# Saguaro-Biosciences/image-processing-suite

Hardware: AMD Instinct MI355X
Metric: fields-of-view/sec, 2080x2080x5ch illum+seg+feat pipe (higher is better)
Workload: dtype fp32 planes / fp64 QC+features / fp32 CPnet (split-fp16 MFMA, f16x3); 1 GPU; configs[1]: 384-well plate, 1 FOV/well, 2080x2080x5ch, illum->seg->feat; batch_per_gpu=48, H=2080, W=2080, C=5, cellpose_model=nuclei, cpnet_weights=cpnet_nuclei_synth.pt, tiles_per_fov=9, parallelism=fov-sharded x1, scheduler=static per-rank steps, steps_this_rank=30, batches_in_flight_per_gpu=2

## Files before the change

image-processing-suite_amd/cpx/_lib.py:

```python
from __future__ import annotations

import ctypes as ct
import os
import threading

_HERE = os.path.dirname(os.path.abspath(__file__))
LIB_PATH = os.environ.get("CPX_LIB", os.path.join(_HERE, "libcpx.so"))

CPX_OK = 0
CPX_DTYPE_NONE, CPX_DTYPE_F32, CPX_DTYPE_F64, CPX_DTYPE_IMAGE_F64 = 0, 1, 2, 3
CPX_QC_OK, CPX_QC_FLAT, CPX_QC_NAN = 0, 1, 2

N_SHAPE = 15
N_INT = 5
N_TEX_PROPS = 6
N_ANGLES = 4
N_TEX = N_TEX_PROPS * N_ANGLES
FEATURES_PER_CHANNEL = N_INT + N_TEX
TEX_DISTANCE = 3


class CpxError(RuntimeError):
    """A libcpx entry point returned a non-zero status."""

# ... 84 lines not shown
    "cpx_seg_average": (_I, [_P, _P, _I, _I, _I, _P, _P, _P]),
    "cpx_embed_preprocess": (_I, [_P, _P, _P, _I, _I, _I, ct.c_float, ct.c_float, _P]),
    "cpx_effnet_stem": (_I, [_P, _P, _I, _I, _I, _P, _P, _P, _P]),
    "cpx_effnet_conv": (_I, [_P, _P, _I, _I, _I, _I, _I, _I, _I, _P, _P, _P, _I, _P, _P, _P]),
    "cpx_effnet_dw": (_I, [_P, _P, _I, _I, _I, _I, _I, _P, _P, _P, _P, _P]),
    "cpx_effnet_dw_blocks": (_I, [_I, _I, _I]),
    "cpx_effnet_se": (_I, [_P, _P, _I, _I, _I, _I, _I, _P, _P, _P, _P, _P]),
    "cpx_effnet_pool": (_I, [_P, _P, _I, _I, _I, _P]),
    "cpx_seg_masks": (_I, [_P, _P, _I, _P, _I, _I, _I, ct.c_double, _I, _I, _I, _P, _P]),
    "cpx_cpnet_epilogue": (_I, [_P, _P, _P, _P, _I, _P, _P, _P, _I, _I, _I, _I, _I, _P, _P, _I]),
    "cpx_cpnet_pool": (_I, [_P, _P, _P, _P, _I, _I, _I, _I, _I, _P, _P]),
    "cpx_cpnet_conv_cfg": (_I, [_I, _I, _P, _P]),
    "cpx_set_illum": (_I, [_P, _I, _P, _I, _I, _I]),
    "cpx_fov_submit": (_I, [_P, ct.c_int64, _P, _I, _I, _I, _I]),
    "cpx_fov_qc": (_I, [_P, _P, _P, _P]),
    "cpx_fov_planes": (_I, [_P, _P, _P]),
    "cpx_fov_read_plane": (_I, [_P, _I, _P]),
    "cpx_fov_segment_post": (_I, [_P, _P, _I, _P, _P, _I, ct.c_double, _I, _I, _I, _P, _P]),
    "cpx_fov_object_table": (_I, [_P, _P, _I, _I, _P, _P]),
    "cpx_fov_features": (_I, [_P, _P, _I, _P, _P]),
    "cpx_fov_wait": (_I, [_P]),
    "cpx_cpnet_conv3x3": (_I, [_P, _P, _I, _I, _I, _I, _I, _P, _P, _P, _I, _P, _P, _P, _I, _P, _P, _I]),
    "cpx_cpnet_conv3x3_head": (_I, [_P, _P, _I, _I, _I, _I, _I, _P, _P, _P, _I, _P, _P, _P, _I, _P,
                                    _P, _P, _I, _P]),
    "cpx_cpnet_stem": (_I, [_P, _P, _I, _I, _I, _P, _P, _P, _P, _P, _P, _P, _P, _P]),
    "cpx_cpnet_x3_cfg": (_I, [_I, _I, _I, _I, _P]),
    "cpx_cpnet_x3_conv": (_I, [_P, _I, _I, _P, _I, _I, _I, _I, _I, _I, _P, _P, _P, _I, _P, _I, _P, _P, _I,
                               _P, _P, _I, _P, _P, _I, _P, _P]),
    "cpx_cpnet_x3_conv_proj": (_I, [_P, _I, _P, _I, _I, _I, _I, _I, _P, _P, _I, _P, _P, _P, _I, _P, _P, _I,
                                    _P, _P, _I, _P]),
    "cpx_cpnet_x3_conv_pool": (_I, [_P, _I, _P, _I, _I, _I, _I, _I, _P, _P, _P, _P, _P, _P, _P, _P, _P]),
    "cpx_cpnet_x3_mask_overflow": (_I, [_P, _P, _I, _I, _I, _I, _P]),
    "cpx_cpnet_x3_stem": (_I, [_P, _P, _I, _I, _I, _P, _P, _P, _P, _P, _P, _P, _P, _P, _P]),
    "cpx_cpnet_x3_pool": (_I, [_P, _P, _P, _P, _I, _I, _I, _I, _I, _P, _P, _P]),
    "cpx_cpnet_x3_style": (_I, [_P, _P, _I, _I, _I, _I, _P, _P, _I, _P]),
}

_lib = None
_lock = threading.Lock()


def load(path: str | None = None):
    global _lib
    with _lock:
        if _lib is not None:
            return _lib
        p = path or LIB_PATH
        try:
            import torch
        except ImportError:
            pass
        if not os.path.exists(p):
            raise CpxNativeMissing(
                f"libcpx.so not found at {p}; build it with `python -c 'import __graft_entry__ as g; g.build()'`")
        try:
            lib = ct.CDLL(p)
        except OSError as e:
            raise CpxNativeMissing(f"failed to load {p}: {e}") from e
        for name, (res, args) in SIGNATURES.items():
            fn = getattr(lib, name)
            fn.restype = res
            fn.argtypes = args
        _lib = lib
        return lib


# ... 9 lines not shown
```

image-processing-suite_amd/cpx/cpnet_x3.py:

```python
from __future__ import annotations

import ctypes as ct

import numpy as np
import torch

from ._lib import check
from .cpnet import CPnet

X3_VARIANT = 0
X3_ZVARIANT = 3
X3_POOL_FUSE = True
X3_FOLD = True


def split_f16(w: np.ndarray):
    w = np.asarray(w, np.float32)
    if not np.all(np.abs(w) < 65504.0):
        raise ValueError("weights outside the fp16 range cannot be split")
    hi = w.astype(np.float16)
    lo = ((w - hi.astype(np.float32)) * np.float32(2048.0)).astype(np.float16)
    return hi, lo


def join_f16(hi: np.ndarray, lo: np.ndarray) -> np.ndarray:
    return (hi.astype(np.float32) + lo.astype(np.float32) * np.float32(1.0 / 2048.0)).astype(np.float32)


def pack_conv(w: np.ndarray, bm: int) -> np.ndarray:
    cout, cin, ks, _ = w.shape
    hi, lo = split_f16(w)
    parts = []
    for a in (hi, lo):
        t = a.reshape(cout // bm, bm, cin // 16, 16, ks, ks).transpose(0, 2, 4, 5, 1, 3)
        parts.append(t)
    return np.ascontiguousarray(np.stack(parts, axis=-2))


def to_split(x: np.ndarray) -> np.ndarray:
    hi, lo = split_f16(x)
    s = x.shape[:-1] + (x.shape[-1] // 16, 16)
    return np.ascontiguousarray(np.stack([hi.reshape(s), lo.reshape(s)], axis=-2))


def from_split(t: np.ndarray) -> np.ndarray:
    if t.dtype != np.float16:
# ... 143 lines not shown

    def _conv_pool(self, x, pk, cout, bias, res, bn):
        N, H, W, cin = x.shape
        yo = self._empty(N, H, W, cout)
        xo = self._empty(N, H // 2, W // 2, cout)
        zo = self._empty(N, H // 2, W // 2, cout)
        check(self.lib.cpx_cpnet_x3_conv_pool(
            self.dev.h, self.variant, _p(x), N, H, W, cin, cout, _p(pk), _p(bias), _p(res), _p(yo), _p(xo), _p(zo),
            _p(bn[0]), _p(bn[1]), self._ovf_p(N)), "cpx_cpnet_x3_conv_pool")
        return yo, xo, zo

    def _proj(self, x, blk):
        return self._conv(x, blk["wp"], blk["cout"], None, ks=1, relu=False, y=True, z=False)[0]

    def _pool(self, x, bn):
        N, H, W, C = x.shape
        xo = self._empty(N, H // 2, W // 2, C)
        zo = self._empty(N, H // 2, W // 2, C)
        scale, shift = bn
        check(self.lib.cpx_cpnet_x3_pool(self.dev.h, _p(x), _p(scale), _p(shift), 1, N, H // 2, W // 2, C,
                                         _p(xo), _p(zo), self._ovf_p(N)), "cpx_cpnet_x3_pool")
        return xo, zo

    def _stem(self, x, d):
        N, H, W, _ = x.shape
        p = self._empty(N, H, W, 32)
        z = self._empty(N, H, W, 32)
        (s0, h0), (s1, h1) = d["bn"][0], d["bn"][1]
        check(self.lib.cpx_cpnet_x3_stem(self.dev.h, _p(x), N, H, W, _p(s0), _p(h0), _p(d["stem_w"]),
                                         _p(d["b"][0]), _p(s1), _p(h1), _p(d["stem_wp"]), _p(p), _p(z),
                                         self._ovf_p(N)), "cpx_cpnet_x3_stem")
        return p, z

    def _style(self, x):
        N, H, W, C = x.shape
        S = torch.empty((N, self.J), dtype=torch.float32, device=self.td)
        check(self.lib.cpx_cpnet_x3_style(self.dev.h, _p(x), N, H, W, C, _p(self.lin_w), _p(self.lin_b),
                                          self.J, _p(S)), "cpx_cpnet_x3_style")
        return S

    @torch.no_grad()
    def __call__(self, x):
        self.dev._bind_stream()
        assert x.dtype == torch.float32 and x.is_contiguous() and x.shape[-1] == 2
        if self.ovf.numel() != x.shape[0]:
            self.ovf = torch.zeros(x.shape[0], dtype=torch.int32, device=self.td)
        self.ovf.zero_()
        xd = []
        zu = None
        nd = len(self.down)
        pooled = None
        for n, d in enumerate(self.down):
            if n == 0:
                p, z = self._stem(x, d)
                x1, z = self._conv(z, d["pk"][1], d["cout"], d["b1p"], res=p, bn=d["bn"][2], y=True)
            else:
                xin, z0 = pooled if pooled is not None else self._pool(xd[-1], d["bn"][0])
                _, z = self._conv(z0, d["pk"][0], d["cout"], d["b"][0], bn=d["bn"][1])
                if d["wpf"] is not None:
                    x1, z = self._conv_proj(z, d["pk"][1], d["cout"], d["b1p"], xin, d["wpf"], bn=d["bn"][2])
                else:
                    p = self._proj(xin, d)
                    x1, z = self._conv(z, d["pk"][1], d["cout"], d["b1p"], res=p, bn=d["bn"][2], y=True)
            _, z = self._conv(z, d["pk"][2], d["cout"], d["b"][2], bn=d["bn"][3])
            if n < nd - 1 and X3_POOL_FUSE:
                xo, xin_n, z0_n = self._conv_pool(z, d["pk"][3], d["cout"], d["b"][3], x1, self.down[n + 1]["bn"][0])
                pooled = (xin_n, z0_n)
            elif n < nd - 1:
                xo, _ = self._conv(z, d["pk"][3], d["cout"], d["b"][3], res=x1, y=True, z=False)
            else:
                xo, zu = self._conv(z, d["pk"][3], d["cout"], d["b"][3], res=x1, bn=self.up[-1]["bn"][0], y=True)
            xd.append(xo)
        S = self._style(xd[-1])
        J = self.J
        x_small, z0 = xd[-1], zu
        for n in range(len(self.up) - 1, -1, -1):
            u = self.up[n]
            so = self.style_off[n]
            sty = [(ct.c_void_p(S.data_ptr() + 4 * o), J) for o in so]
            p = None if u["wpf"] is not None else self._proj(x_small, u)
            _, z = self._conv(z0, u["pk"][0], u["cout"], u["b"][0], res=xd[n], style=sty[0], bn=u["bn"][1],
                              in_up=(n < len(self.up) - 1))
            if p is None:
                x1, z = self._conv_proj(z, u["pk"][1], u["cout"], u["b1p"], x_small, u["wpf"], style=sty[1],
                                        bn=u["bn"][2])
            else:
# ... 13 lines not shown
```

image-processing-suite_amd/csrc/k_conv_x3.hip:

```cpp
#include "cpx_internal.h"
#include <type_traits>
#include <stdlib.h>

namespace {

typedef _Float16 f16x8 __attribute__((ext_vector_type(8)));
typedef _Float16 f16x4 __attribute__((ext_vector_type(4)));
typedef float f32x16 __attribute__((ext_vector_type(16)));

constexpr float kLoScale = 2048.0f;
constexpr float kLoInv = 1.0f / 2048.0f;

typedef __attribute__((address_space(3))) void lds_void_t;
typedef __attribute__((address_space(1))) void glb_void_t;

__device__ uint4 g_x3_zero16 = {0u, 0u, 0u, 0u};

__device__ __forceinline__ int swz4(int row) { return (row >> 2) & 3; }

template <int Q>
__device__ __forceinline__ int swzq(int row) {
  if constexpr (Q >= 16) return row & 15;
  else if constexpr (Q == 8) return (row >> 1) & 7;
  else if constexpr (Q == 4) return (row >> 2) & 3;
// ... 2 lines not shown

__device__ __forceinline__ void split4(float a, float b, float c, float d, uint2& hi, uint2& lo, bool& bad) {
  const float v[4] = {a, b, c, d};
  f16x4 h, l;
#pragma unroll
  for (int k = 0; k < 4; ++k) {
    bad |= !(fabsf(v[k]) < 65504.0f);
    const float vc = fminf(fmaxf(v[k], -65504.0f), 65504.0f);
    const _Float16 t = (_Float16)vc;
    h[k] = t;
    l[k] = (_Float16)((vc - (float)t) * kLoScale);
  }
  hi = __builtin_bit_cast(uint2, h);
  lo = __builtin_bit_cast(uint2, l);
}

__device__ __forceinline__ void join4(const uint2& hi, const uint2& lo, float* out) {
  const f16x4 h = __builtin_bit_cast(f16x4, hi), l = __builtin_bit_cast(f16x4, lo);
#pragma unroll
  for (int k = 0; k < 4; ++k) out[k] = (float)h[k] + (float)l[k] * kLoInv;
}

__device__ __forceinline__ void join8(const uint4& hi, const uint4& lo, float* out) {
  join4(make_uint2(hi.x, hi.y), make_uint2(lo.x, lo.y), out);
  join4(make_uint2(hi.z, hi.w), make_uint2(lo.z, lo.w), out + 4);
}

__device__ __forceinline__ void split8(const float* v, uint4& hi, uint4& lo, bool& bad) {
  uint2 h0, l0, h1, l1;
  split4(v[0], v[1], v[2], v[3], h0, l0, bad);
  split4(v[4], v[5], v[6], v[7], h1, l1, bad);
  hi = make_uint4(h0.x, h0.y, h1.x, h1.y);
  lo = make_uint4(l0.x, l0.y, l1.x, l1.y);
}


struct X3Epi {
  const float* bias;
  const uint4* res;
  const float* style;
  const float* scale;
  const float* shift;
  uint4* y;
  uint4* z;
  int res_up, relu, z_up, style_stride;
  const float* head_w;
  const float* head_b;
  float* head;
  int n_head;
  int* ovf;
  int in_up;
  const uint4* in2;
  const uint4* wpk2;
  uint4* pool_x;
  uint4* pool_z;
  const float* pool_scale;
  const float* pool_shift;
};

template <int COUT, int BM, int TY, int TX, int WM, int WN>
__device__ __forceinline__ void x3_epilogue(f32x16 (&acc0)[WM][WN], const X3Epi& ep, uint4* smem, int n,
                                            int nb, int ty0, int tx0, int H, int W, int mw, int pg, int nsub,
                                            int tid = -1, uint4* res_lds = nullptr) {
  if (tid < 0) tid = threadIdx.x;
  uint4* const ybuf = smem;
  uint4* const zbuf = (res_lds && ep.y) ? res_lds : smem;
  constexpr int NT = 512;
  constexpr int P = TY * TX;
  constexpr int QB = BM / 4;
  constexpr int QC = COUT / 4;
  constexpr int OUT_R = (P * QB + NT - 1) / NT;
  const int lane = threadIdx.x & 63;
  const int h = lane >> 5, l32 = lane & 31;
  bool bad = false;
  auto gpix = [&](int px) -> long long {
    const int gy = ty0 + px / TX, gx = tx0 + px % TX;
    if (px >= P || gy >= H || gx >= W) return -1;
    return ((long long)n * H + gy) * W + gx;
  };
  auto slice = [&](int m) { return mw * WM + m; };
  auto piece = [&](const uint4* buf, int px, int m, int g, int lo) -> uint2* {
    const int q = (slice(m) * 2 + (g >> 1)) * 4 + 2 * lo + (g & 1);
    return reinterpret_cast<uint2*>(const_cast<uint4*>(buf) + px * QB + (q ^ swzq<QB>(px))) + h;
  };
  auto chan = [&](int m, int g) { return nb * BM + slice(m) * 32 + 8 * g + 4 * h; };
  if (ep.bias) {
#pragma unroll
    for (int m = 0; m < WM; ++m)
#pragma unroll
      for (int g = 0; g < 4; ++g) {
        const float4 bv = *reinterpret_cast<const float4*>(ep.bias + chan(m, g));
#pragma unroll
        for (int j = 0; j < WN; ++j) {
          acc0[m][j][4 * g + 0] += bv.x;
          acc0[m][j][4 * g + 1] += bv.y;
          acc0[m][j][4 * g + 2] += bv.z;
          acc0[m][j][4 * g + 3] += bv.w;
        }
      }
  }
  if (ep.res) {
    const uint4* rbuf = res_lds ? res_lds : smem;
    if (!res_lds) {
#pragma unroll
      for (int r = 0; r < OUT_R; ++r) {
        const int i = tid + r * NT;
        if (i < P * QB) {
          const int px = i / QB, k = i - px * QB;
          const int gy = ty0 + px / TX, gx = tx0 + px % TX;
          uint4 v = {0u, 0u, 0u, 0u};
          if (gy < H && gx < W) {
            const long long rp = ep.res_up ? ((long long)n * (H >> 1) + (gy >> 1)) * (W >> 1) + (gx >> 1)
                                           : ((long long)n * H + gy) * W + gx;
            v = ep.res[rp * QC + nb * QB + k];
          }
          smem[px * QB + (k ^ swzq<QB>(px))] = v;
        }
      }
      __syncthreads();
    }
#pragma unroll
    for (int j = 0; j < WN; ++j) {
      const int px = min((pg * WN + j) * 32 + l32, P - 1);
#pragma unroll
      for (int m = 0; m < WM; ++m)
#pragma unroll
        for (int g = 0; g < 4; ++g) {
          float rv[4];
          join4(*piece(rbuf, px, m, g, 0), *piece(rbuf, px, m, g, 1), rv);
#pragma unroll
          for (int k = 0; k < 4; ++k) acc0[m][j][4 * g + k] += rv[k];
        }
    }
    if (!res_lds) __syncthreads();
  }
  auto stage = [&](uint4* buf) {
// ... 433 lines not shown
#pragma unroll
              for (int m = 0; m < WM; ++m) {
                acc0[m][j] = __builtin_amdgcn_mfma_f32_32x32x16_f16(ah[m], bh, acc0[m][j], 0, 0, 0);
                acc1[m][j] = __builtin_amdgcn_mfma_f32_32x32x16_f16(ah[m], bl, acc1[m][j], 0, 0, 0);
                acc1[m][j] = __builtin_amdgcn_mfma_f32_32x32x16_f16(al[m], bh, acc1[m][j], 0, 0, 0);
              }
            }
          }
        }
      });
    }
    if (NBUF == 1) {
      __syncthreads();
      if (ch + 1 < NCHT) issue(ch + 1, 0);
    }
    asm volatile("s_waitcnt vmcnt(0)" ::: "memory");
    __syncthreads();
  }

#pragma unroll
  for (int m = 0; m < WM; ++m)
#pragma unroll
    for (int j = 0; j < WN; ++j)
#pragma unroll
      for (int r = 0; r < 16; ++r) acc0[m][j][r] += acc1[m][j][r] * kLoInv;

  if constexpr (kResPre)
    x3_epilogue<COUT, BM, TY, TX, WM, WN>(acc0, ep, bufO, n, nb, ty0, tx0, H, W, mw, pg, nsub, -1,
                                          ep.res ? bufR : nullptr);
  else
    x3_epilogue<COUT, BM, TY, TX, WM, WN>(acc0, ep, smem, n, nb, ty0, tx0, H, W, mw, pg, nsub);
}

template <int kP32Touch>
__global__ __launch_bounds__(512) __attribute__((amdgpu_waves_per_eu(4)))
void k_conv_x3_p32(const uint4* __restrict__ in, const uint4* __restrict__ wpk, X3Epi ep, int N, int H,
                   int W, int tiles_x, int tiles_y) {
  constexpr int NWV = 8, BM = 32, T = 9, TY = 8, TX = 32, HX = TX + 2, NPIX = (TY + 2) * HX;
  constexpr int NCH = 2, QI = 8;
  constexpr int SW = T * BM * 4;
  constexpr int SI = (NPIX * 4 + 63) / 64 * 64;
  constexpr int NWW = NCH * SW / 64, NWIN = SI / 64;
  constexpr int JW = (NWW + NWV - 1) / NWV, JI = (NWIN + NWV - 1) / NWV;
  static_assert(TY * TX * (BM / 4) <= NCH * SI, "the epilogue stages in the halo buffer");
  static_assert((NCH * SW + NCH * SI) * 16 <= 81920, "two blocks per CU");
  __shared__ uint4 smem[NCH * SW + NCH * SI];
  uint4* sx = smem + NCH * SW;
  const int lane = threadIdx.x & 63, wid = threadIdx.x >> 6;
  const int h = lane >> 5, l32 = lane & 31;
  const int tiles = tiles_x * tiles_y, total = N * tiles;
  const int G = gridDim.x, xb = blockIdx.x & 7, ng = G < 8 ? G : 8;
  const int lo = (int)((long long)total * xb / ng), hi = (int)((long long)total * (xb + 1) / ng);
  const int nbx = (G - xb + 7) >> 3;
  const int fW = (lane & ~3) | ((lane & 3) ^ ((lane >> 4) & 3));
#pragma unroll
  for (int jj = 0; jj < JW; ++jj) {
    const int j = wid + NWV * jj;
    if (j < NWW)
      __builtin_amdgcn_global_load_lds((glb_void_t*)(wpk + j * 64 + fW), (lds_void_t*)(smem + j * 64), 16, 0, 0);
  }
  unsigned touch = 0;
  const int aS = l32 * 4 + (h ^ swz4(l32));
  const int px = wid * 32 + l32;
  const int hp0 = (px / TX) * HX + (px % TX);
  for (int t = lo + (blockIdx.x >> 3); t < hi; t += nbx) {
    const int n = t / tiles, tt = t - n * tiles;
    const int ty0 = (tt / tiles_x) * TY, tx0 = (tt % tiles_x) * TX;
    const uint4* inb = in + (long long)n * H * W * QI;
#pragma unroll
    for (int jj = 0; jj < JI; ++jj) {
      const int j = wid + NWV * jj;
      if (j < NWIN) {
        const int si = j * 64 + lane;
        const int hp = si >> 2, cq = si & 3;
        const int hy = hp / HX, hx = hp - (hp / HX) * HX;
        const int gy = ty0 + hy - 1, gx = tx0 + hx - 1;
        const int off = (hp < NPIX && (unsigned)gy < (unsigned)H && (unsigned)gx < (unsigned)W)
                            ? (gy * W + gx) * QI + (cq ^ swz4(hp)) : -1;
#pragma unroll
        for (int s = 0; s < NCH; ++s) {
          const uint4* src = off >= 0 ? inb + off + s * 4 : &g_x3_zero16;
          __builtin_amdgcn_global_load_lds((glb_void_t*)src, (lds_void_t*)(sx + s * SI + j * 64), 16, 0, 0);
        }
      }
    }
    asm volatile("s_waitcnt vmcnt(0)" ::: "memory");
    __syncthreads();
    unsigned tv0 = 0, tv1 = 0;
    if (kP32Touch) {
      const int i = threadIdx.x;
      if (ep.res && i < TY * TX) {
        const int gy = ty0 + i / TX, gx = tx0 + i % TX;
        if (gy < H && gx < W) {
          const long long rp = ep.res_up ? ((long long)n * (H >> 1) + (gy >> 1)) * (W >> 1) + (gx >> 1)
                                         : ((long long)n * H + gy) * W + gx;
          tv0 = reinterpret_cast<const unsigned*>(ep.res + rp * QI)[0];
        }
      }
      const int t2 = t + nbx;
      if (kP32Touch == 1 && t2 < hi && i < NPIX) {
        const int n2 = t2 / tiles, tt2 = t2 - n2 * tiles;
        const int gy = (tt2 / tiles_x) * TY + i / HX - 1, gx = (tt2 % tiles_x) * TX + i % HX - 1;
        if ((unsigned)gy < (unsigned)H && (unsigned)gx < (unsigned)W)
          tv1 = reinterpret_cast<const unsigned*>(in + ((long long)n2 * H * W + gy * W + gx) * QI)[0];
      }
    }
    int hpb = hp0, aSb = aS;
    asm volatile("" : "+v"(hpb), "+v"(aSb));
    f32x16 acc0[1][1], acc1;
#pragma unroll
    for (int r = 0; r < 16; ++r) {
      acc0[0][0][r] = 0.0f;
      acc1[r] = 0.0f;
    }
#pragma unroll 1
    for (int s = 0; s < NCH; ++s) {
#pragma unroll
      for (int tap = 0; tap < T; ++tap) {
        const int ky = tap / 3, kx = tap % 3;
        const uint4* swt = smem + s * SW + tap * BM * 4;
        const f16x8 ah = __builtin_bit_cast(f16x8, swt[aSb]);
        const f16x8 al = __builtin_bit_cast(f16x8, swt[aSb ^ 2]);
        const int hp = hpb + ky * HX + kx;
        const int bs = s * SI + hp * 4 + (h ^ swz4(hp));
        const f16x8 bh = __builtin_bit_cast(f16x8, sx[bs]);
        const f16x8 bl = __builtin_bit_cast(f16x8, sx[bs ^ 2]);
        acc0[0][0] = __builtin_amdgcn_mfma_f32_32x32x16_f16(ah, bh, acc0[0][0], 0, 0, 0);
        acc1 = __builtin_amdgcn_mfma_f32_32x32x16_f16(ah, bl, acc1, 0, 0, 0);
        acc1 = __builtin_amdgcn_mfma_f32_32x32x16_f16(al, bh, acc1, 0, 0, 0);
      }
      x3_sched();
    }
#pragma unroll
    for (int r = 0; r < 16; ++r) acc0[0][0][r] += acc1[r] * kLoInv;
    __syncthreads();
    X3Epi et = ep;
    int zo = 0;
    asm volatile("" : "+s"(zo));
    et.bias = et.bias ? et.bias + zo : nullptr;
    et.scale = et.scale ? et.scale + zo : nullptr;
    et.shift = et.shift ? et.shift + zo : nullptr;
    et.style = et.style ? et.style + zo : nullptr;
    et.head_w = et.head_w ? et.head_w + zo : nullptr;
    et.head_b = et.head_b ? et.head_b + zo : nullptr;
    int tid = threadIdx.x;
    asm volatile("" : "+v"(tid));
    x3_epilogue<32, BM, TY, TX, 1, 1>(acc0, et, sx, n, 0, ty0, tx0, H, W, 0, wid, 1, tid);
    touch ^= tv0 ^ tv1;
    __syncthreads();
  }
  if (kP32Touch && N < 0 && touch == 0x9e3779b9u) ep.ovf[0] = 1;
}

struct X3Cfg {
  int bm, ty, tx;
};

bool x3_cfg(int ks, int cin, int cout, int variant, X3Cfg* c) {
  if (!((cin == 32 || cin == 64 || cin == 128 || cin == 256) && (cout == 32 || cout == 64 || cout == 128 || cout == 256)))
    return false;
  if (ks == 1) {
    *c = {32, 16, 16};
    return true;
  }
  if (ks != 3) return false;
  if (cout == 32) *c = variant == 1 ? X3Cfg{32, 16, 32} : X3Cfg{32, 8, 32};
  else if (cout == 64) *c = variant == 1 ? X3Cfg{64, 16, 16} : variant == 2 ? X3Cfg{32, 16, 32}
                          : variant == 3 ? X3Cfg{64, 16, 16} : X3Cfg{32, 16, 16};
  else *c = variant == 1 ? X3Cfg{64, 14, 28} : variant == 2 ? X3Cfg{32, 16, 28}
          : variant == 3 ? X3Cfg{64, 8, 28} : X3Cfg{32, 8, 28};
  return true;
}

template <int KS, int CIN, int COUT, int BM, int TY, int TX, int WM, int WN, int WPE, int CIN2 = 0, int NBUF = 2>
int x3_run(cpx_ctx* ctx, const void* in, const void* wpk, const X3Epi& ep, int N, int H, int W) {
  const int tx = cpx_div_up(W, TX), ty = cpx_div_up(H, TY);
  const long long blocks = (long long)N * tx * ty * (COUT / BM);
  CPX_REQUIRE(blocks < (1LL << 31), CPX_ERR_ARG, "cpx_cpnet_x3_conv: too many tiles");
  hipLaunchKernelGGL((k_conv_x3<KS, CIN, COUT, BM, TY, TX, WM, WN, WPE, CIN2, NBUF>), dim3((unsigned)blocks),
                     dim3(512), 0, ctx->stream, (const uint4*)in, (const uint4*)wpk, ep, N, H, W, tx, ty);
// ... 13 lines not shown
#define X3_P1(CI, CO, C2, V, BM_, TY_, TX_, WM_, WN_, WPE_)                               \
  if (cin == CI && cout == CO && cin2 == C2 && variant == V)                               \
    return x3_run<3, CI, CO, BM_, TY_, TX_, WM_, WN_, WPE_, C2, 1>(ctx, in, wpk, ep, N, H, W);
  X3_P1(64, 64, 32, 2, 32, 16, 32, 1, 2, 4)
  X3_P1(128, 128, 64, 2, 32, 16, 28, 1, 2, 4)
  X3_P1(256, 256, 128, 2, 32, 16, 28, 1, 2, 4)
  X3_P1(256, 256, 256, 2, 32, 16, 28, 1, 2, 4)
  X3_P1(64, 64, 32, 3, 64, 16, 16, 2, 1, 4)
  X3_P1(128, 128, 64, 3, 64, 8, 28, 2, 1, 4)
  X3_P1(256, 256, 128, 3, 64, 8, 28, 2, 1, 4)
  X3_P1(256, 256, 256, 3, 64, 8, 28, 2, 1, 4)
#undef X3_P1
#undef X3_P
  cpx_set_error("cpx_cpnet_x3_conv_proj: no instance for %d -> %d channels + projection of %d (variant %d)",
                cin, cout, cin2, variant);
  return CPX_ERR_SHAPE;
}

int x3_launch(cpx_ctx* ctx, int ks, int cin, int cout, int variant, const void* in, const void* wpk,
              const X3Epi& ep, int N, int H, int W) {
#define X3_3(CI, CO, V, BM_, TY_, TX_, WM_, WN_, WPE_)                                  \
  if (ks == 3 && cin == CI && cout == CO && variant == V)                                \
    return x3_run<3, CI, CO, BM_, TY_, TX_, WM_, WN_, WPE_>(ctx, in, wpk, ep, N, H, W);
#define X3_1(CI, CO)                                                                     \
  if (ks == 1 && cin == CI && cout == CO)                                                \
    return x3_run<1, CI, CO, 32, 16, 16, 1, 1, 4>(ctx, in, wpk, ep, N, H, W);
  if ((variant == 2 || variant == 3) && cout == 32) variant = 0;
  if (ks == 3 && cin == 32 && cout == 32 && variant == 0 && !ep.in_up) {
    const int tx = cpx_div_up(W, 32), ty = cpx_div_up(H, 8);
    const long long tiles = (long long)N * tx * ty;
    CPX_REQUIRE(tiles < (1LL << 31), CPX_ERR_ARG, "cpx_cpnet_x3_conv: too many tiles");
    const int grid = (int)std::max(1LL, std::min(tiles, 2LL * ctx->n_cu));
    hipLaunchKernelGGL(k_conv_x3_p32<2>, dim3(grid), dim3(512), 0, ctx->stream, (const uint4*)in, (const uint4*)wpk, ep, N,
                       H, W, tx, ty);
    CPX_CHECK_LAUNCH("k_conv_x3_p32");
    return CPX_OK;
  }
#define X3_3B(CI, CO, V, BM_, TY_, TX_, WM_, WN_, WPE_)                                  \
  if (ks == 3 && cin == CI && cout == CO && variant == V)                                \
    return x3_run<3, CI, CO, BM_, TY_, TX_, WM_, WN_, WPE_, 0, 1>(ctx, in, wpk, ep, N, H, W);
  X3_3B(32, 64, 2, 32, 16, 32, 1, 2, 4)
  X3_3B(64, 64, 2, 32, 16, 32, 1, 2, 4)
  X3_3B(128, 64, 2, 32, 16, 32, 1, 2, 4)
  X3_3B(64, 128, 2, 32, 16, 28, 1, 2, 4)
  X3_3B(128, 128, 2, 32, 16, 28, 1, 2, 4)
  X3_3B(256, 128, 2, 32, 16, 28, 1, 2, 4)
  X3_3B(128, 256, 2, 32, 16, 28, 1, 2, 4)
  X3_3B(256, 256, 2, 32, 16, 28, 1, 2, 4)
  X3_3B(32, 64, 3, 64, 16, 16, 2, 1, 4)
  X3_3B(64, 64, 3, 64, 16, 16, 2, 1, 4)
  X3_3B(128, 64, 3, 64, 16, 16, 2, 1, 4)
  X3_3B(64, 128, 3, 64, 8, 28, 2, 1, 4)
  X3_3B(128, 128, 3, 64, 8, 28, 2, 1, 4)
  X3_3B(256, 128, 3, 64, 8, 28, 2, 1, 4)
  X3_3B(128, 256, 3, 64, 8, 28, 2, 1, 4)
  X3_3B(256, 256, 3, 64, 8, 28, 2, 1, 4)
#undef X3_3B
  X3_3(32, 32, 0, 32, 8, 32, 1, 1, 4)
  X3_3(64, 32, 0, 32, 8, 32, 1, 1, 4)
  X3_3(32, 32, 1, 32, 16, 32, 1, 2, 2)
  X3_3(64, 32, 1, 32, 16, 32, 1, 2, 2)
  X3_3(32, 64, 1, 64, 16, 16, 2, 1, 2)
  X3_3(64, 64, 1, 64, 16, 16, 2, 1, 2)
  X3_3(128, 64, 1, 64, 16, 16, 2, 1, 2)
  X3_3(32, 64, 0, 32, 16, 16, 1, 1, 4)
  X3_3(64, 64, 0, 32, 16, 16, 1, 1, 4)
  X3_3(128, 64, 0, 32, 16, 16, 1, 1, 4)
// ... 10 lines not shown
  X3_1(32, 64)
  X3_1(64, 128)
  X3_1(128, 256)
  X3_1(256, 256)
  X3_1(256, 128)
  X3_1(128, 64)
  X3_1(64, 32)
#undef X3_3
#undef X3_1
  cpx_set_error("cpx_cpnet_x3_conv: no instance for ks %d, %d -> %d channels (variant %d)", ks, cin, cout, variant);
  return CPX_ERR_SHAPE;
}

constexpr int kSTY = 16, kSTX = 16;

__global__ __launch_bounds__(kSTY * kSTX) void k_cpnet_stem_x3(
    const float* __restrict__ x, int N, int H, int W, const float* __restrict__ scale0,
    const float* __restrict__ shift0, const float* __restrict__ w0, const float* __restrict__ bias0,
    const float* __restrict__ scale1, const float* __restrict__ shift1, const float* __restrict__ wp,
    uint4* __restrict__ p_out, uint4* __restrict__ z_out, int tiles_x, int tiles_y, int* ovf) {
  constexpr int NP = kSTY * kSTX;
  __shared__ float sz[2][kSTY + 2][kSTX + 2];
  __shared__ uint4 so[2][NP * 8];
  const int tiles = tiles_x * tiles_y;
  const int n = blockIdx.x / tiles, t = blockIdx.x - n * tiles;
  const int ty0 = (t / tiles_x) * kSTY, tx0 = (t % tiles_x) * kSTX;
  const float s00 = scale0[0], s01 = scale0[1], h00 = shift0[0], h01 = shift0[1];
  for (int i = threadIdx.x; i < (kSTY + 2) * (kSTX + 2); i += NP) {
    const int hy = i / (kSTX + 2), hx = i - hy * (kSTX + 2);
    const int gy = ty0 + hy - 1, gx = tx0 + hx - 1;
    float a = 0.0f, b = 0.0f;
    if (gy >= 0 && gy < H && gx >= 0 && gx < W) {
      const float2 v = *reinterpret_cast<const float2*>(x + (((long long)n * H + gy) * W + gx) * 2);
      a = fmaxf(s00 * v.x + h00, 0.0f);
      b = fmaxf(s01 * v.y + h01, 0.0f);
    }
    sz[0][hy][hx] = a;
    sz[1][hy][hx] = b;
  }
  __syncthreads();
  const int ly = threadIdx.x / kSTX, lx = threadIdx.x - ly * kSTX;
  const int gy = ty0 + ly, gx = tx0 + lx;
  bool bad = false;
  const int px = threadIdx.x;
  if (gy < H && gx < W) {
    const long long pix = ((long long)n * H + gy) * W + gx;
    float in[18];
#pragma unroll
    for (int c = 0; c < 2; ++c)
#pragma unroll
      for (int k = 0; k < 9; ++k) in[c * 9 + k] = sz[c][ly + k / 3][lx + k % 3];
    const float2 xv = *reinterpret_cast<const float2*>(x + pix * 2);
#pragma unroll
    for (int q = 0; q < 4; ++q) {
      float zf[8], pf[8];
#pragma unroll
      for (int e = 0; e < 8; ++e) {
        const int co = q * 8 + e;
        float acc = 0.0f;
#pragma unroll
        for (int k = 0; k < 18; ++k) acc = __builtin_fmaf(w0[co * 18 + k], in[k], acc);
        zf[e] = fmaxf(__builtin_fmaf(scale1[co], acc + bias0[co], shift1[co]), 0.0f);
        pf[e] = __builtin_fmaf(wp[co * 2], xv.x, wp[co * 2 + 1] * xv.y);
      }
      uint4 hi, lo;
      const int base = (q >> 1) * 4 + (q & 1);
      split8(zf, hi, lo, bad);
      so[0][px * 8 + (base ^ (px & 7))] = hi;
      so[0][px * 8 + ((base + 2) ^ (px & 7))] = lo;
      split8(pf, hi, lo, bad);
      so[1][px * 8 + (base ^ (px & 7))] = hi;
      so[1][px * 8 + ((base + 2) ^ (px & 7))] = lo;
    }
  }
  __syncthreads();
#pragma unroll
  for (int r = 0; r < 8; ++r) {
    const int i = threadIdx.x + r * NP;
    const int p = i >> 3, k = i & 7;
    const int py = ty0 + p / kSTX, pxg = tx0 + p % kSTX;
    if (py < H && pxg < W) {
      const long long g = (((long long)n * H + py) * W + pxg) * 8 + k;
      z_out[g] = so[0][p * 8 + (k ^ (p & 7))];
      p_out[g] = so[1][p * 8 + (k ^ (p & 7))];
    }
  }
  if (ovf && __ballot(bad) && (threadIdx.x & 63) == 0) atomicOr(ovf + n, 1);
}

__global__ __launch_bounds__(256) void k_cpnet_pool_x3(const uint4* __restrict__ in,
                                                       const float* __restrict__ scale,
                                                       const float* __restrict__ shift, int relu,
                                                       int N, int Hh, int Ww, int Cn,
                                                       uint4* __restrict__ xo, uint4* __restrict__ zo,
                                                       int* ovf) {
  const long long P = (long long)Hh * Ww;
  const int G = Cn / 8;
// ... 186 lines not shown
  CPX_REQUIRE(N > 0 && H > 0 && W > 0 && cin2 > 0 && cin2 % 16 == 0, CPX_ERR_ARG, "cpx_cpnet_x3_conv_proj: bad sizes");
  CPX_REQUIRE(!(scale == nullptr) == !(shift == nullptr), CPX_ERR_ARG,
              "cpx_cpnet_x3_conv_proj: scale and shift go together");
  CPX_REQUIRE(((uintptr_t)in | (uintptr_t)wpk | (uintptr_t)in2 | (uintptr_t)wpk2 | (uintptr_t)y_out |
               (uintptr_t)z_out) % 16 == 0, CPX_ERR_ARG, "cpx_cpnet_x3_conv_proj: misaligned buffers");
  CPX_REQUIRE(!style || (style_stride >= cout && style_stride % 4 == 0 && ((uintptr_t)style % 16) == 0),
              CPX_ERR_ARG, "cpx_cpnet_x3_conv_proj: style needs a 16-byte aligned [N][stride >= cout] table");
  CPX_REQUIRE(!z_up || z_out, CPX_ERR_ARG, "cpx_cpnet_x3_conv_proj: z_up without z_out");
  X3Epi ep{bias, nullptr, style, scale, shift, (uint4*)y_out, (uint4*)z_out, 0, relu, z_up, style_stride,
           nullptr, nullptr, nullptr, 0, ovf, 0, (const uint4*)in2, (const uint4*)wpk2,
           nullptr, nullptr, nullptr, nullptr};
  return x3_launch_proj(ctx, cin, cout, cin2, variant, in, wpk, ep, N, H, W);
}

extern "C" int cpx_cpnet_x3_stem(cpx_ctx* ctx, const float* x, int N, int H, int W,
                                 const float* scale0, const float* shift0, const float* w0,
                                 const float* bias0, const float* scale1, const float* shift1,
                                 const float* wp, void* p_out, void* z_out, int* ovf) {
  CPX_REQUIRE(ctx && x && scale0 && shift0 && w0 && bias0 && scale1 && shift1 && wp && p_out && z_out,
              CPX_ERR_ARG, "cpx_cpnet_x3_stem: null argument");
  CPX_REQUIRE(N > 0 && H > 0 && W > 0, CPX_ERR_ARG, "cpx_cpnet_x3_stem: bad sizes");
  CPX_REQUIRE(((uintptr_t)x % 8) == 0 && ((uintptr_t)p_out | (uintptr_t)z_out) % 16 == 0,
              CPX_ERR_ARG, "cpx_cpnet_x3_stem: misaligned buffers");
  const int tx = cpx_div_up(W, kSTX), ty = cpx_div_up(H, kSTY);
  const long long blocks = (long long)N * tx * ty;
  CPX_REQUIRE(blocks < (1LL << 31), CPX_ERR_ARG, "cpx_cpnet_x3_stem: too many tiles");
  hipLaunchKernelGGL(k_cpnet_stem_x3, dim3((unsigned)blocks), dim3(kSTY * kSTX), 0, ctx->stream, x, N, H,
                     W, scale0, shift0, w0, bias0, scale1, shift1, wp, (uint4*)p_out, (uint4*)z_out, tx,
                     ty, ovf);
  CPX_CHECK_LAUNCH("k_cpnet_stem_x3");
  return CPX_OK;
}

extern "C" int cpx_cpnet_x3_pool(cpx_ctx* ctx, const void* in, const float* scale,
                                 const float* shift, int relu, int N, int Hh, int Ww, int Cn,
                                 void* x_out, void* z_out, int* ovf) {
  CPX_REQUIRE(ctx && in && (x_out || z_out), CPX_ERR_ARG, "cpx_cpnet_x3_pool: null argument");
  CPX_REQUIRE(N > 0 && Hh > 0 && Ww > 0 && Cn > 0 && Cn % 16 == 0, CPX_ERR_ARG,
              "cpx_cpnet_x3_pool: bad sizes (channels must be a multiple of 16)");
  CPX_REQUIRE(!(scale == nullptr) == !(shift == nullptr), CPX_ERR_ARG,
              "cpx_cpnet_x3_pool: scale and shift go together");
  CPX_REQUIRE(((uintptr_t)in | (uintptr_t)x_out | (uintptr_t)z_out) % 16 == 0, CPX_ERR_ARG,
              "cpx_cpnet_x3_pool: buffers must be 16-byte aligned");
  const long long ng = (long long)N * Hh * Ww * Cn / 8;
  const long long g = std::max(1LL, std::min((ng + 255) / 256, 32LL * ctx->n_cu));
  hipLaunchKernelGGL(k_cpnet_pool_x3, dim3((unsigned)g), dim3(256), 0, ctx->stream, (const uint4*)in,
                     scale, shift, relu, N, Hh, Ww, Cn, (uint4*)x_out, (uint4*)z_out, ovf);
  CPX_CHECK_LAUNCH("k_cpnet_pool_x3");
  return CPX_OK;
}

extern "C" int cpx_cpnet_x3_style(cpx_ctx* ctx, const void* x, int N, int H, int W, int C,
                                  const float* lin_w, const float* lin_b, int J, float* out) {
  CPX_REQUIRE(ctx && x && lin_w && lin_b && out, CPX_ERR_ARG, "cpx_cpnet_x3_style: null argument");
  CPX_REQUIRE(N > 0 && H > 0 && W > 0 && C > 0 && C <= 256 && C % 16 == 0 && J > 0, CPX_ERR_ARG,
              "cpx_cpnet_x3_style: bad sizes");
  hipLaunchKernelGGL(k_cpnet_style_x3, dim3(N), dim3(256), 0, ctx->stream, (const uint4*)x, H, W, C,
                     lin_w, lin_b, J, out);
  CPX_CHECK_LAUNCH("k_cpnet_style_x3");
  return CPX_OK;
}
```

include/cpx.h:

```cpp
#ifndef CPX_H
#define CPX_H

#include <stdint.h>

#ifdef __cplusplus
extern "C" {
#endif

#define CPX_ABI_VERSION 1

#define CPX_OK 0
#define CPX_ERR_ARG 1
#define CPX_ERR_HIP 2
#define CPX_ERR_SHAPE 3
#define CPX_ERR_OOM 4
#define CPX_ERR_STATE 5

#define CPX_DTYPE_NONE 0
#define CPX_DTYPE_F32 1
#define CPX_DTYPE_F64 2
#define CPX_DTYPE_IMAGE_F64 3

typedef struct cpx_ctx cpx_ctx;

// ... 220 lines not shown
                   int relu, int N, int Hh, int Ww, int Cn, void* x_out, void* z_out);
int cpx_cpnet_conv_cfg(int cin, int cout, int* bn, int* ck);
int cpx_cpnet_conv3x3(cpx_ctx* ctx, const void* in, int N, int H, int W, int cin, int cout,
                      const void* wpk, const float* bias, const void* res, int res_up,
                      const float* style, const float* scale, const float* shift, int relu,
                      void* y_out, void* z_out, int z_up);
int cpx_cpnet_conv3x3_head(cpx_ctx* ctx, const void* in, int N, int H, int W, int cin, int cout,
                           const void* wpk, const float* bias, const void* res, int res_up,
                           const float* style, const float* scale, const float* shift, int relu,
                           void* y_out, const float* head_w, const float* head_b, int n_head,
                           void* head_out);
int cpx_cpnet_stem(cpx_ctx* ctx, const void* x, int N, int H, int W, const float* scale0,
                   const float* shift0, const float* w0, const float* bias0, const float* scale1,
                   const float* shift1, const float* wp, void* p_out, void* z_out);

int cpx_cpnet_x3_cfg(int ks, int cin, int cout, int variant, int* bm);
int cpx_cpnet_x3_conv(cpx_ctx* ctx, int ks, int variant, const void* in, int in_up, int N, int H,
                      int W, int cin, int cout, const void* wpk, const float* bias, const void* res,
                      int res_up, const float* style, int style_stride, const float* scale,
                      const float* shift, int relu, void* y_out, void* z_out, int z_up,
                      const float* head_w, const float* head_b, int n_head, float* head_out,
                      int* ovf);
int cpx_cpnet_x3_conv_proj(cpx_ctx* ctx, int variant, const void* in, int N, int H, int W, int cin,
                           int cout, const void* wpk, const void* in2, int cin2, const void* wpk2,
                           const float* bias, const float* style, int style_stride, const float* scale,
                           const float* shift, int relu, void* y_out, void* z_out, int z_up, int* ovf);
int cpx_cpnet_x3_conv_pool(cpx_ctx* ctx, int variant, const void* in, int N, int H, int W, int cin,
                           int cout, const void* wpk, const float* bias, const void* res, void* y_out,
                           void* pool_x, void* pool_z, const float* pool_scale, const float* pool_shift,
                           int* ovf);
int cpx_cpnet_x3_stem(cpx_ctx* ctx, const float* x, int N, int H, int W, const float* scale0,
                      const float* shift0, const float* w0, const float* bias0, const float* scale1,
                      const float* shift1, const float* wp, void* p_out, void* z_out, int* ovf);
int cpx_cpnet_x3_pool(cpx_ctx* ctx, const void* in, const float* scale, const float* shift,
                      int relu, int N, int Hh, int Ww, int Cn, void* x_out, void* z_out, int* ovf);
int cpx_cpnet_x3_mask_overflow(cpx_ctx* ctx, float* out, int N, int H, int W, int nout, const int* ovf);
int cpx_cpnet_x3_style(cpx_ctx* ctx, const void* x, int N, int H, int W, int C, const float* lin_w,
                       const float* lin_b, int J, float* out);

#define CPX_QC_OK 0
#define CPX_QC_FLAT 1
#define CPX_QC_NAN 2

int cpx_set_illum(cpx_ctx* ctx, int ch, const void* host, int dtype, int H, int W);
int cpx_fov_submit(cpx_ctx* ctx, int64_t site_id, const uint16_t* const* planes, int C, int Z,
                   int H, int W);
int cpx_fov_qc(cpx_ctx* ctx, double* slope_out, double* pctmax_out, int* status);
int cpx_fov_planes(cpx_ctx* ctx, const float** corr_dev, const uint16_t** plane_dev);
int cpx_fov_read_plane(cpx_ctx* ctx, int ch, uint16_t* host);
int cpx_fov_segment_post(cpx_ctx* ctx, const void* net_dev, int layout, const cpx_seg_geom* geom,
                         const float* taper_dev, int niter, double flow_threshold, int min_size,
                         int max_objects, int resample, int32_t* labels_dev,
                         cpx_seg_stats* stats_dev);
int cpx_fov_object_table(cpx_ctx* ctx, const int32_t* labels_dev, int box, int max_objects,
                    cpx_object* host_out, int* n_out);
int cpx_fov_features(cpx_ctx* ctx, const int32_t* labels_dev, int max_objects, double* host_out,
                     int* n_out);
int cpx_fov_wait(cpx_ctx* ctx);

int cpx_debug_glcm_timing(cpx_ctx* ctx, int enable);
int cpx_debug_glcm_ms(cpx_ctx* ctx, double* ms_out, int* launches_out);
int cpx_debug_seg_timing(cpx_ctx* ctx, int enable);
int cpx_debug_seg_stats(cpx_ctx* ctx, double* follow_ms, double* item_steps, double* fe_reg_ms, int* calls);
int cpx_debug_flow_error_counts(cpx_ctx* ctx, int out[8]);
int cpx_debug_flow_error_class(int bh, int bw);

// ... 8 lines not shown
```

Measured before the change: 503.2 FOV/s.

## Fuse CPnet stem into first x3 conv kernel, recomputing stem on halo

Adds a stem-fused variant of the 32-channel x3 conv kernel. The stem's 3x3 conv, BN and ReLU are computed directly into LDS for each tile plus its halo, and the 1x1 projection residual is recomputed in the epilogue from the raw input. This removes the separate stem launch and the global write and read of the intermediate p/z tensors. In exchange the stem is recomputed on halo pixels, the conv prologue becomes ALU-heavy instead of an async global-to-LDS copy, and it is only used when variant != 1.

Result: no change. 504.3 FOV/s, median of 6 (+0.2%).

```diff
diff --git a/image-processing-suite_amd/cpx/_lib.py b/image-processing-suite_amd/cpx/_lib.py
--- a/image-processing-suite_amd/cpx/_lib.py
+++ b/image-processing-suite_amd/cpx/_lib.py
@@ -140,6 +140,7 @@
     "cpx_cpnet_x3_conv_pool": (_I, [_P, _I, _P, _I, _I, _I, _I, _I, _P, _P, _P, _P, _P, _P, _P, _P, _P]),
     "cpx_cpnet_x3_mask_overflow": (_I, [_P, _P, _I, _I, _I, _I, _P]),
     "cpx_cpnet_x3_stem": (_I, [_P, _P, _I, _I, _I, _P, _P, _P, _P, _P, _P, _P, _P, _P, _P]),
+    "cpx_cpnet_x3_conv_stem": (_I, [_P, _P, _I, _I, _I, _P, _P, _P, _P, _P, _P, _P, _P, _P, _P, _P, _P, _P, _P]),
     "cpx_cpnet_x3_pool": (_I, [_P, _P, _P, _P, _I, _I, _I, _I, _I, _P, _P, _P]),
     "cpx_cpnet_x3_style": (_I, [_P, _P, _I, _I, _I, _I, _P, _P, _I, _P]),
 }
diff --git a/image-processing-suite_amd/cpx/cpnet_x3.py b/image-processing-suite_amd/cpx/cpnet_x3.py
--- a/image-processing-suite_amd/cpx/cpnet_x3.py
+++ b/image-processing-suite_amd/cpx/cpnet_x3.py
@@ -12,6 +12,7 @@
 X3_ZVARIANT = 3
 X3_POOL_FUSE = True
 X3_FOLD = True
+X3_STEM_FUSE = True
 
 
 def split_f16(w: np.ndarray):
@@ -221,6 +222,17 @@
                                          self._ovf_p(N)), "cpx_cpnet_x3_stem")
         return p, z
 
+    def _conv_stem(self, x, d):
+        N, H, W, _ = x.shape
+        yo = self._empty(N, H, W, 32)
+        zo = self._empty(N, H, W, 32)
+        (s0, h0), (s1, h1), (s2, h2) = d["bn"][0], d["bn"][1], d["bn"][2]
+        check(self.lib.cpx_cpnet_x3_conv_stem(
+            self.dev.h, _p(x), N, H, W, _p(s0), _p(h0), _p(d["stem_w"]), _p(d["b"][0]), _p(s1), _p(h1),
+            _p(d["stem_wp"]), _p(d["pk"][1]), _p(d["b1p"]), _p(s2), _p(h2), _p(yo), _p(zo), self._ovf_p(N)),
+            "cpx_cpnet_x3_conv_stem")
+        return yo, zo
+
     def _style(self, x):
         N, H, W, C = x.shape
         S = torch.empty((N, self.J), dtype=torch.float32, device=self.td)
@@ -240,7 +252,9 @@
         nd = len(self.down)
         pooled = None
         for n, d in enumerate(self.down):
-            if n == 0:
+            if n == 0 and X3_STEM_FUSE and self.variant != 1:
+                x1, z = self._conv_stem(x, d)
+            elif n == 0:
                 p, z = self._stem(x, d)
                 x1, z = self._conv(z, d["pk"][1], d["cout"], d["b1p"], res=p, bn=d["bn"][2], y=True)
             else:
diff --git a/image-processing-suite_amd/csrc/k_conv_x3.hip b/image-processing-suite_amd/csrc/k_conv_x3.hip
--- a/image-processing-suite_amd/csrc/k_conv_x3.hip
+++ b/image-processing-suite_amd/csrc/k_conv_x3.hip
@@ -58,6 +58,51 @@
   split4(v[4], v[5], v[6], v[7], h1, l1, bad);
   hi = make_uint4(h0.x, h0.y, h1.x, h1.y);
   lo = make_uint4(l0.x, l0.y, l1.x, l1.y);
+}
+
+struct X3Stem {
+  const float* x;
+  const float* scale0;
+  const float* shift0;
+  const float* w0;
+  const float* bias0;
+  const float* scale1;
+  const float* shift1;
+  const float* wp;
+};
+
+typedef const __attribute__((address_space(4))) float* x3_cfp;
+__device__ __forceinline__ x3_cfp x3_const(const float* p) { return (x3_cfp)p; }
+
+__device__ __forceinline__ float2 stem_z0(float2 v, float s00, float s01, float h00, float h01) {
+  return make_float2(fmaxf(s00 * v.x + h00, 0.0f), fmaxf(s01 * v.y + h01, 0.0f));
+}
+
+template <class TP>
+__device__ __forceinline__ void stem_z8(const float (&in)[18], TP w0, TP bias0, TP scale1, TP shift1, int c0,
+                                        float (&zf)[8]) {
+  typedef float f32x2 __attribute__((ext_vector_type(2)));
+#pragma unroll
+  for (int e = 0; e < 8; e += 2) {
+    const int co = c0 + e;
+    f32x2 acc = {0.0f, 0.0f};
+#pragma unroll
+    for (int k = 0; k < 18; ++k) {
+      const f32x2 w = {w0[co * 18 + k], w0[(co + 1) * 18 + k]}, v = {in[k], in[k]};
+      acc = __builtin_elementwise_fma(w, v, acc);
+    }
+    zf[e] = fmaxf(__builtin_fmaf(scale1[co], acc.x + bias0[co], shift1[co]), 0.0f);
+    zf[e + 1] = fmaxf(__builtin_fmaf(scale1[co + 1], acc.y + bias0[co + 1], shift1[co + 1]), 0.0f);
+  }
+}
+
+template <class TP>
+__device__ __forceinline__ void stem_p8(float2 xv, TP wp, int c0, float (&pf)[8]) {
+#pragma unroll
+  for (int e = 0; e < 8; ++e) {
+    const int co = c0 + e;
+    pf[e] = __builtin_fmaf(wp[co * 2], xv.x, wp[co * 2 + 1] * xv.y);
+  }
 }
 
 
@@ -84,10 +129,11 @@
   const float* pool_shift;
 };
 
-template <int COUT, int BM, int TY, int TX, int WM, int WN>
+template <int COUT, int BM, int TY, int TX, int WM, int WN, bool STEM = false>
 __device__ __forceinline__ void x3_epilogue(f32x16 (&acc0)[WM][WN], const X3Epi& ep, uint4* smem, int n,
                                             int nb, int ty0, int tx0, int H, int W, int mw, int pg, int nsub,
-                                            int tid = -1, uint4* res_lds = nullptr) {
+                                            int tid = -1, uint4* res_lds = nullptr,
+                                            const X3Stem* st = nullptr) {
   if (tid < 0) tid = threadIdx.x;
   uint4* const ybuf = smem;
   uint4* const zbuf = (res_lds && ep.y) ? res_lds : smem;
@@ -125,9 +171,29 @@
         }
       }
   }
-  if (ep.res) {
+  if (STEM || ep.res) {
     const uint4* rbuf = res_lds ? res_lds : smem;
-    if (!res_lds) {
+    if constexpr (STEM) {
+      static_assert(COUT == 32 && BM == 32 && P % 128 == 0 && NT == 512, "stem-fed residual");
+      const int wv = __builtin_amdgcn_readfirstlane(threadIdx.x >> 6);
+      const int q = wv & 3, base = (q >> 1) * 4 + (q & 1);
+      const float* xb = st->x + (long long)n * H * W * 2;
+#pragma unroll
+      for (int r = 0; r < P / 128; ++r) {
+        const int px = (wv >> 2) * (P / 2) + r * 64 + lane;
+        const int gy = ty0 + px / TX, gx = tx0 + px % TX;
+        uint4 hi = {0u, 0u, 0u, 0u}, lo = {0u, 0u, 0u, 0u};
+        if (gy < H && gx < W) {
+          const float2 xv = *reinterpret_cast<const float2*>(xb + ((long long)gy * W + gx) * 2);
+          float pf[8];
+          stem_p8(xv, x3_const(st->wp), q * 8, pf);
+          split8(pf, hi, lo, bad);
+        }
+        smem[px * QB + (base ^ swzq<QB>(px))] = hi;
+        smem[px * QB + ((base + 2) ^ swzq<QB>(px))] = lo;
+      }
+      __syncthreads();
+    } else if (!res_lds) {
 #pragma unroll
       for (int r = 0; r < OUT_R; ++r) {
         const int i = tid + r * NT;
@@ -627,10 +693,12 @@
     x3_epilogue<COUT, BM, TY, TX, WM, WN>(acc0, ep, smem, n, nb, ty0, tx0, H, W, mw, pg, nsub);
 }
 
-template <int kP32Touch>
+struct X3NoStem {};
+
+template <int kP32Touch, bool kStem = false>
 __global__ __launch_bounds__(512) __attribute__((amdgpu_waves_per_eu(4)))
 void k_conv_x3_p32(const uint4* __restrict__ in, const uint4* __restrict__ wpk, X3Epi ep, int N, int H,
-                   int W, int tiles_x, int tiles_y) {
+                   int W, int tiles_x, int tiles_y, std::conditional_t<kStem, X3Stem, X3NoStem> st) {
   constexpr int NWV = 8, BM = 32, T = 9, TY = 8, TX = 32, HX = TX + 2, NPIX = (TY + 2) * HX;
   constexpr int NCH = 2, QI = 8;
   constexpr int SW = T * BM * 4;
@@ -662,20 +730,72 @@
     const int n = t / tiles, tt = t - n * tiles;
     const int ty0 = (tt / tiles_x) * TY, tx0 = (tt % tiles_x) * TX;
     const uint4* inb = in + (long long)n * H * W * QI;
-#pragma unroll
-    for (int jj = 0; jj < JI; ++jj) {
-      const int j = wid + NWV * jj;
-      if (j < NWIN) {
-        const int si = j * 64 + lane;
-        const int hp = si >> 2, cq = si & 3;
-        const int hy = hp / HX, hx = hp - (hp / HX) * HX;
-        const int gy = ty0 + hy - 1, gx = tx0 + hx - 1;
-        const int off = (hp < NPIX && (unsigned)gy < (unsigned)H && (unsigned)gx < (unsigned)W)
-                            ? (gy * W + gx) * QI + (cq ^ swz4(hp)) : -1;
-#pragma unroll
-        for (int s = 0; s < NCH; ++s) {
-          const uint4* src = off >= 0 ? inb + off + s * 4 : &g_x3_zero16;
-          __builtin_amdgcn_global_load_lds((glb_void_t*)src, (lds_void_t*)(sx + s * SI + j * 64), 16, 0, 0);
+    if constexpr (kStem) {
+      static_assert(NPIX % 2 == 0 && NPIX / 2 <= 3 * 64, "two half-halos of three 64-lane rounds");
+      const int wv = __builtin_amdgcn_readfirstlane(wid);
+      const int q = wv & 3;
+      const float2* xb = reinterpret_cast<const float2*>(st.x) + (long long)n * H * W;
+      const x3_cfp sc0 = x3_const(st.scale0), sh0 = x3_const(st.shift0);
+      const float s00 = sc0[0], s01 = sc0[1], h00 = sh0[0], h01 = sh0[1];
+      bool bad = false;
+#pragma unroll 1
+      for (int r = 0; r < 3; ++r) {
+        int zo = 0;
+        asm volatile("" : "+s"(zo));
+        const int hl = r * 64 + lane;
+        if (hl < NPIX / 2) {
+          const int hp = (wv >> 2) * (NPIX / 2) + hl;
+          const int hy = hp / HX, hx = hp - hy * HX;
+          const int gy = ty0 + hy - 1, gx = tx0 + hx - 1;
+          uint4 zh = {0u, 0u, 0u, 0u}, zl = {0u, 0u, 0u, 0u};
+          if ((unsigned)gy < (unsigned)H && (unsigned)gx < (unsigned)W) {
+            float2 xv[9];
+#pragma unroll
+            for (int k = 0; k < 9; ++k) {
+              const int yc = min(max(gy + k / 3 - 1, 0), H - 1), xc = min(max(gx + k % 3 - 1, 0), W - 1);
+              xv[k] = xb[yc * W + xc];
+            }
+            asm volatile("" : "+v"(xv[0].x), "+v"(xv[0].y), "+v"(xv[1].x), "+v"(xv[1].y), "+v"(xv[2].x),
+                         "+v"(xv[2].y), "+v"(xv[3].x), "+v"(xv[3].y), "+v"(xv[4].x), "+v"(xv[4].y),
+                         "+v"(xv[5].x), "+v"(xv[5].y), "+v"(xv[6].x), "+v"(xv[6].y), "+v"(xv[7].x),
+                         "+v"(xv[7].y), "+v"(xv[8].x), "+v"(xv[8].y));
+            float zin[18];
+#pragma unroll
+            for (int k = 0; k < 9; ++k) {
+              const int yy = gy + k / 3 - 1, xx = gx + k % 3 - 1;
+              const float2 a = stem_z0(xv[k], s00, s01, h00, h01);
+              const bool inside = (unsigned)yy < (unsigned)H && (unsigned)xx < (unsigned)W;
+              zin[k] = inside ? a.x : 0.0f;
+              zin[9 + k] = inside ? a.y : 0.0f;
+            }
+            float zf[8];
+            stem_z8(zin, x3_const(st.w0 + zo), x3_const(st.bias0 + zo), x3_const(st.scale1 + zo),
+                    x3_const(st.shift1 + zo), q * 8, zf);
+            split8(zf, zh, zl, bad);
+          }
+          sx[(q >> 1) * SI + hp * 4 + ((q & 1) ^ swz4(hp))] = zh;
+          sx[(q >> 1) * SI + hp * 4 + (((q & 1) + 2) ^ swz4(hp))] = zl;
+        }
+      }
+      if (ep.ovf && __ballot(bad)) {
+        if (lane == 0) atomicOr(ep.ovf + n, 1);
+      }
+    } else {
+#pragma unroll
+      for (int jj = 0; jj < JI; ++jj) {
+        const int j = wid + NWV * jj;
+        if (j < NWIN) {
+          const int si = j * 64 + lane;
+          const int hp = si >> 2, cq = si & 3;
+          const int hy = hp / HX, hx = hp - (hp / HX) * HX;
+          const int gy = ty0 + hy - 1, gx = tx0 + hx - 1;
+          const int off = (hp < NPIX && (unsigned)gy < (unsigned)H && (unsigned)gx < (unsigned)W)
+                              ? (gy * W + gx) * QI + (cq ^ swz4(hp)) : -1;
+#pragma unroll
+          for (int s = 0; s < NCH; ++s) {
+            const uint4* src = off >= 0 ? inb + off + s * 4 : &g_x3_zero16;
+            __builtin_amdgcn_global_load_lds((glb_void_t*)src, (lds_void_t*)(sx + s * SI + j * 64), 16, 0, 0);
+          }
         }
       }
     }
@@ -740,7 +860,13 @@
     et.head_b = et.head_b ? et.head_b + zo : nullptr;
     int tid = threadIdx.x;
     asm volatile("" : "+v"(tid));
-    x3_epilogue<32, BM, TY, TX, 1, 1>(acc0, et, sx, n, 0, ty0, tx0, H, W, 0, wid, 1, tid);
+    if constexpr (kStem) {
+      X3Stem se = st;
+      se.wp = se.wp + zo;
+      x3_epilogue<32, BM, TY, TX, 1, 1, true>(acc0, et, sx, n, 0, ty0, tx0, H, W, 0, wid, 1, tid, nullptr, &se);
+    } else {
+      x3_epilogue<32, BM, TY, TX, 1, 1>(acc0, et, sx, n, 0, ty0, tx0, H, W, 0, wid, 1, tid);
+    }
     touch ^= tv0 ^ tv1;
     __syncthreads();
   }
@@ -820,7 +946,7 @@
     CPX_REQUIRE(tiles < (1LL << 31), CPX_ERR_ARG, "cpx_cpnet_x3_conv: too many tiles");
     const int grid = (int)std::max(1LL, std::min(tiles, 2LL * ctx->n_cu));
     hipLaunchKernelGGL(k_conv_x3_p32<2>, dim3(grid), dim3(512), 0, ctx->stream, (const uint4*)in, (const uint4*)wpk, ep, N,
-                       H, W, tx, ty);
+                       H, W, tx, ty, X3NoStem{});
     CPX_CHECK_LAUNCH("k_conv_x3_p32");
     return CPX_OK;
   }
@@ -897,8 +1023,9 @@
     float a = 0.0f, b = 0.0f;
     if (gy >= 0 && gy < H && gx >= 0 && gx < W) {
       const float2 v = *reinterpret_cast<const float2*>(x + (((long long)n * H + gy) * W + gx) * 2);
-      a = fmaxf(s00 * v.x + h00, 0.0f);
-      b = fmaxf(s01 * v.y + h01, 0.0f);
+      const float2 z0 = stem_z0(v, s00, s01, h00, h01);
+      a = z0.x;
+      b = z0.y;
     }
     sz[0][hy][hx] = a;
     sz[1][hy][hx] = b;
@@ -919,15 +1046,8 @@
 #pragma unroll
     for (int q = 0; q < 4; ++q) {
       float zf[8], pf[8];
-#pragma unroll
-      for (int e = 0; e < 8; ++e) {
-        const int co = q * 8 + e;
-        float acc = 0.0f;
-#pragma unroll
-        for (int k = 0; k < 18; ++k) acc = __builtin_fmaf(w0[co * 18 + k], in[k], acc);
-        zf[e] = fmaxf(__builtin_fmaf(scale1[co], acc + bias0[co], shift1[co]), 0.0f);
-        pf[e] = __builtin_fmaf(wp[co * 2], xv.x, wp[co * 2 + 1] * xv.y);
-      }
+      stem_z8(in, w0, bias0, scale1, shift1, q * 8, zf);
+      stem_p8(xv, wp, q * 8, pf);
       uint4 hi, lo;
       const int base = (q >> 1) * 4 + (q & 1);
       split8(zf, hi, lo, bad);
@@ -1180,6 +1300,30 @@
   return CPX_OK;
 }
 
+extern "C" int cpx_cpnet_x3_conv_stem(cpx_ctx* ctx, const float* x, int N, int H, int W, const float* scale0,
+                                      const float* shift0, const float* w0, const float* bias0,
+                                      const float* scale1, const float* shift1, const float* wp,
+                                      const void* wpk, const float* bias, const float* scale,
+                                      const float* shift, void* y_out, void* z_out, int* ovf) {
+  CPX_REQUIRE(ctx && x && scale0 && shift0 && w0 && bias0 && scale1 && shift1 && wp && wpk && bias && scale &&
+                  shift && y_out && z_out, CPX_ERR_ARG, "cpx_cpnet_x3_conv_stem: null argument");
+  CPX_REQUIRE(N > 0 && H > 0 && W > 0, CPX_ERR_ARG, "cpx_cpnet_x3_conv_stem: bad sizes");
+  CPX_REQUIRE(((uintptr_t)x % 8) == 0 && ((uintptr_t)wpk | (uintptr_t)bias | (uintptr_t)scale | (uintptr_t)shift |
+                                          (uintptr_t)y_out | (uintptr_t)z_out) % 16 == 0,
+              CPX_ERR_ARG, "cpx_cpnet_x3_conv_stem: misaligned buffers");
+  const int tx = cpx_div_up(W, 32), ty = cpx_div_up(H, 8);
+  const long long tiles = (long long)N * tx * ty;
+  CPX_REQUIRE(tiles < (1LL << 31), CPX_ERR_ARG, "cpx_cpnet_x3_conv_stem: too many tiles");
+  X3Epi ep{bias, nullptr, nullptr, scale, shift, (uint4*)y_out, (uint4*)z_out, 0, 1, 0, 0,
+           nullptr, nullptr, nullptr, 0, ovf, 0, nullptr, nullptr, nullptr, nullptr, nullptr, nullptr};
+  const int grid = (int)std::max(1LL, std::min(tiles, 2LL * ctx->n_cu));
+  hipLaunchKernelGGL((k_conv_x3_p32<0, true>), dim3(grid), dim3(512), 0, ctx->stream, (const uint4*)nullptr,
+                     (const uint4*)wpk, ep, N, H, W, tx, ty,
+                     X3Stem{x, scale0, shift0, w0, bias0, scale1, shift1, wp});
+  CPX_CHECK_LAUNCH("k_conv_x3_p32<0, true>");
+  return CPX_OK;
+}
+
 extern "C" int cpx_cpnet_x3_pool(cpx_ctx* ctx, const void* in, const float* scale,
                                  const float* shift, int relu, int N, int Hh, int Ww, int Cn,
                                  void* x_out, void* z_out, int* ovf) {
diff --git a/include/cpx.h b/include/cpx.h
--- a/include/cpx.h
+++ b/include/cpx.h
@@ -276,6 +276,11 @@
 int cpx_cpnet_x3_stem(cpx_ctx* ctx, const float* x, int N, int H, int W, const float* scale0,
                       const float* shift0, const float* w0, const float* bias0, const float* scale1,
                       const float* shift1, const float* wp, void* p_out, void* z_out, int* ovf);
+int cpx_cpnet_x3_conv_stem(cpx_ctx* ctx, const float* x, int N, int H, int W, const float* scale0,
+                           const float* shift0, const float* w0, const float* bias0,
+                           const float* scale1, const float* shift1, const float* wp, const void* wpk,
+                           const float* bias, const float* scale, const float* shift, void* y_out,
+                           void* z_out, int* ovf);
 int cpx_cpnet_x3_pool(cpx_ctx* ctx, const void* in, const float* scale, const float* shift,
                       int relu, int N, int Hh, int Ww, int Cn, void* x_out, void* z_out, int* ovf);
 int cpx_cpnet_x3_mask_overflow(cpx_ctx* ctx, float* out, int N, int H, int W, int nout, const int* ovf);
```
